# fperezgamonal/flownet2-tf

Measured on AMD Instinct MI355X. Metric: forward pairs/sec at 512x384 (FlowNet2), higher is better.
Workload: dtype f16x2 (split fp16 hi+lo operands, 3 fp16 MFMAs per product, fp32 accumulate); 1 GPU; FlowNet2 forward, batch=4 synthetic 512x384 pairs per GPU, seeded synthetic weights; pairs_per_gpu=4, parallelism=dp1 (no collective)

## Files before the change

flownet2-tf_amd/csrc/conv2.hip:

```cpp
#include "conv_common.h"

#include <type_traits>
#include <algorithm>
#include <utility>

#ifndef FN2_X2_ORDER
#define FN2_X2_ORDER 0
#endif
#ifndef FN2_CONV_ABLATE
#define FN2_CONV_ABLATE 0
#endif
#ifndef FN2_SETPRIO
#define FN2_SETPRIO 1
#endif

namespace fn2 {

typedef __attribute__((address_space(3))) void* lptr_t;

constexpr unsigned kOobOffset = 0x80000000u;

typedef int v4i_t __attribute__((ext_vector_type(4)));
typedef unsigned u32x4_t __attribute__((ext_vector_type(4)));

// ... 476 lines not shown
    issue_stage(lds0);
    asm volatile("s_waitcnt vmcnt(0)" ::: "memory");
    __syncthreads();
    const int nst2 = ((kt1 - (kt0 - grp) + KG - 1) / KG + 1) & ~1;
    for (int s = 0; s < nst2; s += 2) {
      issue_stage(lds1);
      compute(lds0);
      asm volatile("s_waitcnt vmcnt(0)" ::: "memory");
      __syncthreads();
      if (s + 2 < nst2) issue_stage(lds0);
      compute(lds1);
      asm volatile("s_waitcnt vmcnt(0)" ::: "memory");
      __syncthreads();
    }
  } else if constexpr (kDeep) {
    constexpr int ND = NWI + NPI, D = STAGES - 1;
    static_assert(ND * (D - 1) <= 63, "vmcnt field");
    auto slot_ptr = [&](int sl) { return lds0_all + sl * (ROWS * 8); };
#pragma unroll
    for (int d = 0; d < D; ++d) issue_stage(slot_ptr(d));
    const int nst = kt1 - kt0;
    int rd = 0, wr = D;
    for (int s = 0; s < nst; ++s) {
      asm volatile("s_waitcnt vmcnt(%0)\n\ts_barrier" :: "n"(ND * (D - 1)) : "memory");
      issue_stage(slot_ptr(wr));
      compute(slot_ptr(rd));
      rd = rd + 1 == STAGES ? 0 : rd + 1;
      wr = wr + 1 == STAGES ? 0 : wr + 1;
    }
    asm volatile("s_waitcnt vmcnt(0)" ::: "memory");
  } else {
    constexpr int ND = NWI + NPI;
    static_assert(ND == 5 || ND == 6 || ND == 8, "vmcnt literal below");
    auto ring_sync = [] {
      if constexpr (ND == 5) asm volatile("s_waitcnt vmcnt(5)\n\ts_barrier" ::: "memory");
      else if constexpr (ND == 6) asm volatile("s_waitcnt vmcnt(6)\n\ts_barrier" ::: "memory");
      else asm volatile("s_waitcnt vmcnt(8)\n\ts_barrier" ::: "memory");
    };
    issue_stage(lds0);
    issue_stage(lds1);
    const int nst3 = (kt1 - kt0 + 2) / 3 * 3;
    for (int s = 0; s < nst3; s += 3) {
      ring_sync(); issue_stage(lds2); compute(lds0);
      ring_sync(); issue_stage(lds0); compute(lds1);
      ring_sync(); issue_stage(lds1); compute(lds2);
    }
    asm volatile("s_waitcnt vmcnt(0)" ::: "memory");
  }

  if constexpr (KG > 1) {
    constexpr int NA4 = TCN * TPN * 4;
    static_assert((KG - 1) * 4 * NA4 * 64 <= KG * ROWS * 8, "reduction scratch must fit the stage buffers");
    float4* red = reinterpret_cast<float4*>(lds0_all);
    auto acc4 = [&](int idx) -> float4 {
      if constexpr (M16) {
        const f32x4 v = acc16[idx / (TPN * 2)][idx % (TPN * 2)];
        return make_float4(v[0], v[1], v[2], v[3]);
      } else {
        const int t = idx >> 2, q = idx & 3;
        return make_float4(acc[t / TPN][t % TPN][4 * q], acc[t / TPN][t % TPN][4 * q + 1], acc[t / TPN][t % TPN][4 * q + 2],
                           acc[t / TPN][t % TPN][4 * q + 3]);
      }
    };
    if (grp > 0) {
#pragma unroll
      for (int idx = 0; idx < NA4; ++idx) red[(((grp - 1) * 4 + wave) * NA4 + idx) * 64 + lane] = acc4(idx);
    }
    __syncthreads();
    if (grp > 0) return;
#pragma unroll
    for (int g = 0; g < KG - 1; ++g)
#pragma unroll
      for (int idx = 0; idx < NA4; ++idx) {
        const float4 v = red[((g * 4 + wave) * NA4 + idx) * 64 + lane];
        if constexpr (M16) {
          f32x4& d = acc16[idx / (TPN * 2)][idx % (TPN * 2)];
          d[0] += v.x; d[1] += v.y; d[2] += v.z; d[3] += v.w;
        } else {
          const int t = idx >> 2, q = idx & 3;
          acc[t / TPN][t % TPN][4 * q] += v.x; acc[t / TPN][t % TPN][4 * q + 1] += v.y;
          acc[t / TPN][t % TPN][4 * q + 2] += v.z; acc[t / TPN][t % TPN][4 * q + 3] += v.w;
        }
      }
  }

  if constexpr (HEAD5) {
    if (p.dbg & 2) return;
    constexpr int TS = 52;
    static_assert(256 * TS * 4 <= 2 * ROWS * 128, "T fits the stage buffers");
#pragma unroll
    for (int tc = 0; tc < TCN; ++tc)
#pragma unroll
      for (int tp = 0; tp < TPN; ++tp) {
        const int pos = wp * TPN * 32 + tp * 32 + fr;
        const int cb = tc * 32 + fh * 16;
#pragma unroll
        for (int q = 0; q < 4; ++q)
          if (cb + 4 * q < TS)
            *reinterpret_cast<float4*>(h5_t(lds0_all, lds1_all, ROWS * 128, pos * TS + cb + 4 * q)) =
                make_float4(acc[tc][tp][4 * q] * p.out_scale, acc[tc][tp][4 * q + 1] * p.out_scale,
                            acc[tc][tp][4 * q + 2] * p.out_scale, acc[tc][tp][4 * q + 3] * p.out_scale);
      }
    __syncthreads();
    if (p.dbg & 8) return;
    const int tx = bx % p.h5_tx, tyn = bx / p.h5_tx;
    const int n = tyn / p.h5_ty, ty = tyn - n * p.h5_ty;
    float* pf = reinterpret_cast<float*>(p.out);
    if (tid < 224) {
      const int o = tid & 1, px = tid >> 1;
      const int py = px / 28, pxx = px - py * 28;
      const int oy = ty * 4 + py, ox = tx * 28 + pxx;
      if (oy < p.OH && ox < p.OW && !(p.h5_ring && (oy == 0 || oy == p.OH - 1 || ox == 0 || ox == p.OW - 1))) {
        float a = p.bias ? p.bias[o] : 0.f;
#pragma unroll
        for (int uy = 0; uy < 5; ++uy)
#pragma unroll
          for (int ux = 0; ux < 5; ++ux)
            a += *h5_t(lds0_all, lds1_all, ROWS * 128, ((py + uy) * 32 + pxx + ux) * TS + (uy * 5 + ux) * 2 + o);
        pf[(((size_t)n * p.OH + oy) * p.OW + ox) * 2 + o] = a;
      }
    }
    return;
  }
  if (FN2_CONV_ABLATE && (p.dbg & 262144)) return;
  if constexpr (M16) {
    OutT* out16 = reinterpret_cast<OutT*>(p.out);
    const int r16 = lane & 15, g16 = lane >> 4;
    float* slab = p.splitk > 1 ? p.ws + (size_t)split * p.N * p.out_H * p.out_W * p.ws_cs : nullptr;
#pragma unroll
    for (int b = 0; b < TPN * 2; ++b) {
      const int m = m0 + wp * TPN * 32 + b * 16 + r16;
      if (m >= p.M) continue;
      const int n = m / (p.OH * p.OW);
      const int rem = m - n * (p.OH * p.OW);
      const int oy = rem / p.OW, ox = rem - oy * p.OW;
      const size_t opix = ((size_t)n * p.out_H + (oy * osc + oy_off)) * p.out_W + (ox * osc + ox_off);
      OutT* po = out16 + opix * p.out_cs + p.out_c0;
#pragma unroll
      for (int a = 0; a < TCN * 2; ++a) {
        const int co = c0 + wc * TCN * 32 + (a >> 1) * 32 + 16 * (g16 & 1) + 8 * (a & 1) + 4 * (g16 >> 1);
        if (slab != nullptr) {
          if (co < p.ws_cs)
            *reinterpret_cast<float4*>(slab + opix * p.ws_cs + co) =
                make_float4(acc16[a][b][0], acc16[a][b][1], acc16[a][b][2], acc16[a][b][3]);
          continue;
        }
        float v[4];
#pragma unroll
        for (int j = 0; j < 4; ++j) {
          float x = acc16[a][b][j] * p.out_scale + ((p.bias != nullptr && co + j < p.Cout) ? p.bias[co + j] : 0.f);
          if constexpr (sizeof(OutT) == 4) {
            if (p.accum && co + j < p.Cout) x += load_elem<OutT>(po + co + j);
            if (co + j < p.Cout) x = act_grad<OutT>(p, out16, po + co + j, co + j, x);
          }
          if (p.act == FN2_ACT_LEAKY) x = leaky(x);
          v[j] = x;
        }
        if (p.vec_ok && co + 3 < p.Cout) store_vec<OutT, 4>(po + co, v);
        else
#pragma unroll
          for (int j = 0; j < 4; ++j)
            if (co + j < p.Cout) store_elem<OutT>(po + co + j, v[j]);
      }
    }
    return;
  }

  OutT* out = reinterpret_cast<OutT*>(p.out);
  constexpr int WCOLS = TCN * 32, RS = WCOLS + 4, WROWS = 32 * TPN;
  constexpr int WTW = WROWS * RS + WROWS;
  constexpr bool kLdsT = (KG > 1 ? 4 : 2) * WTW * 4 <= KG * ROWS * 128;
  if constexpr (FEED && !kLdsT) { if (feeder) return; }
  float* const tl = reinterpret_cast<float*>(KG > 1 ? ep1 : (wave < 2 ? lds0_all : ep1)) + (KG > 1 ? wave : (wave & 1)) * WTW;
  constexpr int CPR = WCOLS / 4, RPI = 64 / CPR;
  static_assert(!SLAB || WREG, "SLAB is a specialisation of the WREG instantiations");
  if ((SLAB || !WREG) && p.splitk > 1) {
    float* slab = p.ws + (size_t)split * p.N * p.out_H * p.out_W * p.ws_cs;
    if constexpr (kLdsT) {
      if constexpr (STAGES >= 3) __syncthreads();
      if constexpr (FEED) { if (feeder) return; }
      int* rowoff = reinterpret_cast<int*>(tl + WROWS * RS);
#pragma unroll
      for (int tp = 0; tp < TPN; ++tp) {
        const int m = m0 + wp * TPN * 32 + tp * 32 + fr;
        const int mm = m < p.M ? m : 0;
        const int n = mm / (p.OH * p.OW);
        const int rem = mm - n * (p.OH * p.OW);
        const int oy = rem / p.OW, ox = rem - oy * p.OW;
        if (fh == 0) rowoff[tp * 32 + fr] = m < p.M ? (int)((((size_t)n * p.out_H + (oy * osc + oy_off)) * p.out_W + (ox * osc + ox_off)) * p.ws_cs) : -1;
#pragma unroll
        for (int tc = 0; tc < TCN; ++tc)
#pragma unroll
          for (int q = 0; q < 4; ++q)
            *reinterpret_cast<float4*>(tl + (tp * 32 + fr) * RS + tc * 32 + fh * 16 + q * 4) =
                make_float4(acc[tc][tp][4 * q], acc[tc][tp][4 * q + 1], acc[tc][tp][4 * q + 2], acc[tc][tp][4 * q + 3]);
      }
      const int rr = lane / CPR, ch = lane - rr * CPR;
      const int co = c0 + wc * WCOLS + ch * 4;
#pragma unroll
      for (int i = 0; i < WROWS / RPI; ++i) {
        const int row = i * RPI + rr;
        const float4 v = *reinterpret_cast<const float4*>(tl + row * RS + ch * 4);
        const int off = rowoff[row];
        if (off >= 0 && co < p.ws_cs) *reinterpret_cast<float4*>(slab + (size_t)off + co) = v;
      }
      return;
    }
#pragma unroll
    for (int tp = 0; tp < TPN; ++tp) {
      const int m = m0 + wp * TPN * 32 + tp * 32 + fr;
      if (m >= p.M) continue;
      const int n = m / (p.OH * p.OW);
      const int rem = m - n * (p.OH * p.OW);
      const int oy = rem / p.OW, ox = rem - oy * p.OW;
      float* po = slab + (((size_t)n * p.out_H + (oy * osc + oy_off)) * p.out_W + (ox * osc + ox_off)) * p.ws_cs;
#pragma unroll
      for (int tc = 0; tc < TCN; ++tc)
#pragma unroll
        for (int q = 0; q < 4; ++q) {
          const int co = c0 + wc * TCN * 32 + tc * 32 + fh * 16 + q * 4;
          if (co < p.ws_cs)
            *reinterpret_cast<float4*>(po + co) = make_float4(acc[tc][tp][4 * q], acc[tc][tp][4 * q + 1],
                                                              acc[tc][tp][4 * q + 2], acc[tc][tp][4 * q + 3]);
        }
    }
    return;
  }
  if constexpr (SLAB) return;
  const bool vec16 = (p.out_cs % 8 == 0) && (p.out_c0 % 8 == 0);
  const bool wide = kLdsT && sizeof(OutT) == 4 && vec16 && c0 + wc * WCOLS + WCOLS <= p.Cout && !(p.dbg & 4194304);
  int* const rowoff = reinterpret_cast<int*>(tl + WROWS * RS);
  if constexpr (STAGES >= 3 && kLdsT) __syncthreads();
  if constexpr (FEED) { if (feeder) return; }
#pragma unroll
  for (int tc = 0; tc < TCN; ++tc) {
    const int cout_base = c0 + wc * TCN * 32 + tc * 32 + fh * 16;
    float bias[16];
#pragma unroll
    for (int q = 0; q < 16; ++q) bias[q] = (p.bias != nullptr && cout_base + q < p.Cout) ? p.bias[cout_base + q] : 0.f;
#pragma unroll
    for (int tp = 0; tp < TPN; ++tp) {
      const int m = m0 + wp * TPN * 32 + tp * 32 + fr;
      if (wide && tc == 0 && fh == 0) rowoff[tp * 32 + fr] = m < p.M ? 0 : -1;
      if (m >= p.M) continue;
      const int n = m / (p.OH * p.OW);
      const int rem = m - n * (p.OH * p.OW);
      const int oy = rem / p.OW, ox = rem - oy * p.OW;
      const size_t opix = (((size_t)n * p.out_H + (oy * osc + oy_off)) * p.out_W + (ox * osc + ox_off));
      OutT* po = out + opix * p.out_cs + p.out_c0 + cout_base;
      float v[16];
#pragma unroll
      for (int q = 0; q < 16; ++q) v[q] = acc[tc][tp][q] * p.out_scale + bias[q];
      accum_act_grad16<OutT>(p, out, po, cout_base, vec16 && cout_base + 15 < p.Cout, v);
      if (p.act == FN2_ACT_LEAKY) {
#pragma unroll
        for (int q = 0; q < 16; ++q) v[q] = leaky(v[q]);
      }
      if (wide) {
        if (tc == 0 && fh == 0) rowoff[tp * 32 + fr] = (int)opix;
        store16<OutT>(reinterpret_cast<OutT*>(tl + (tp * 32 + fr) * RS + tc * 32 + fh * 16), v);
      } else if (vec16 && cout_base + 15 < p.Cout) {
        store16<OutT>(po, v);
      } else {
#pragma unroll
        for (int q = 0; q < 16; ++q)
          if (cout_base + q < p.Cout) store_elem<OutT>(po + q, v[q]);
      }
    }
  }
  if (wide) {
    const int rr = lane / CPR, ch = lane - rr * CPR;
    OutT* ob = out + p.out_c0 + c0 + wc * WCOLS + ch * 4;
#pragma unroll
    for (int i = 0; i < WROWS / RPI; ++i) {
      const int row = i * RPI + rr;
      const uint4 v = *reinterpret_cast<const uint4*>(tl + row * RS + ch * 4);
      const int opix = rowoff[row];
      if (opix >= 0) *reinterpret_cast<uint4*>(ob + (size_t)opix * p.out_cs) = v;
    }
  }
#endif
}

template <typename OutT, int WC, int WP, int TCN, int TPN, int KW>
__global__ void __launch_bounds__(256) conv_halo_kernel(const ConvArgs p) {
#if defined(__HIP_DEVICE_COMPILE__)
  using T = x2_t;
  constexpr int ESZ = 4;
  constexpr int BC = WC * TCN * 32, BP = WP * TPN * 32;
  static_assert(WC * WP == 4, "4 waves per block");
  constexpr int NWI = BC / 32;
  constexpr int BROWS = BP + 8;
  constexpr int NBP = BROWS / 8;
  constexpr int NBW = (NBP + 3) / 4;
  __shared__ uint4 ldsA[2][BC * 8];
  __shared__ uint4 ldsB[2][BROWS * 8];

  const int tid = threadIdx.x, lane = tid & 63;
  const int wave = __builtin_amdgcn_readfirstlane(tid >> 6);
  const int wc = wave / WP, wp = wave % WP;

  int pad_y = p.pad, pad_x = p.pad, oy_off = 0, ox_off = 0, osc = 1;
  const T* wgt = reinterpret_cast<const T*>(p.wgt);
  const int phase = blockIdx.z;
  const unsigned wrow_bytes = (unsigned)p.ksteps * 128u;
  if (p.merged) {
    pad_y = phase ? p.ph_pad1 : p.ph_pad0; pad_x = 1; oy_off = phase; ox_off = 0; osc = 2;
    wgt += (size_t)phase * p.cout_pad * (wrow_bytes / ESZ);
  } else if (p.deconv) {
    const int a = phase >> 1, b = phase & 1;
    pad_y = a ? p.ph_pad1 : p.ph_pad0; pad_x = b ? p.ph_pad1 : p.ph_pad0; oy_off = a; ox_off = b; osc = 2;
    wgt += (size_t)phase * p.cout_pad * (wrow_bytes / ESZ);
  }
  int bx = blockIdx.x, by = blockIdx.y;
  {
    const int NT = gridDim.x * gridDim.y, L = blockIdx.x + gridDim.x * blockIdx.y;
    const int xcd = L & 7, chunk = NT >> 3, rem = NT & 7;
    const int Lp = xcd * chunk + min(xcd, rem) + (L >> 3);
    bx = Lp / (int)gridDim.y;
    by = Lp - bx * (int)gridDim.y;
  }
  const int m0 = bx * BP, c0 = by * BC;
  const int tn = m0 / (p.OH * p.OW);
  const int trem = m0 - tn * (p.OH * p.OW);
  const int toy = trem / p.OW, tox = trem - toy * p.OW;
  const int iy_base = toy - pad_y, ix_base = tox - pad_x;

  const v4i_t rsrc_w = make_rsrc(wgt, (int)(p.cout_pad * wrow_bytes));
  const v4i_t rsrc_x = make_rsrc(p.in, p.in_bytes);
  const int lrow = lane >> 3, lphys = lane & 7;
  unsigned woff[NWI];
#pragma unroll
  for (int j = 0; j < NWI; ++j) {
    const int row = wave * (BC / 4) + j * 8 + lrow;
    woff[j] = (unsigned)(c0 + row) * wrow_bytes + (unsigned)((lphys ^ ((row >> 1) & 7)) * 16);
  }
  int boff[NBW];
  bool bok[NBW];
#pragma unroll
  for (int j = 0; j < NBW; ++j) {
    const int q = wave + 4 * j;
    const int e = q * 8 + lrow;
    const int ix = ix_base + e;
    bok[j] = q < NBP && e < BP + KW - 1 && ix >= 0 && ix < p.W;
    boff[j] = (((tn * p.H + iy_base) * p.W + ix) * p.in_cs + p.in_c0) * ESZ + (lphys ^ ((e >> 1) & 7)) * 16;
  }
  const int spt = p.cin_chunks >> 3;
  const int nsup = spt * p.KH;
  auto issue_B = [&](int sup, uint4* lds) {
    const int sc = sup / p.KH, ky = sup - sc * p.KH;
    const bool yok = (unsigned)(iy_base + ky) < (unsigned)p.H;
    const int toff = (ky * p.W * p.in_cs) * ESZ + sc * 128;
#pragma unroll
    for (int j = 0; j < NBW; ++j) {
      const int q = wave + 4 * j;
      if (q < NBP) dma16(rsrc_x, &lds[q * 64], (bok[j] && yok) ? (unsigned)(boff[j] + toff) : kOobOffset, 0);
    }
  };
  auto issue_A = [&](int sup, int kx, uint4* lds) {
    const int sc = sup / p.KH, ky = sup - sc * p.KH;
    const int soff = ((ky * KW + kx) * spt + sc) * 128;
#pragma unroll
    for (int j = 0; j < NWI; ++j) dma16(rsrc_w, &lds[(wave * (BC / 4) + j * 8) * 8], woff[j], soff);
  };

  const int fr = lane & 31, fh = lane >> 5, fsw = (fr >> 1) & 7;
  f32x16 acc[TCN][TPN];
#pragma unroll
  for (int tc = 0; tc < TCN; ++tc)
#pragma unroll
    for (int tp = 0; tp < TPN; ++tp)
#pragma unroll
      for (int q = 0; q < 16; ++q) acc[tc][tp][q] = 0.f;

  auto compute = [&](const uint4* la, const uint4* lb, int kx) {
#if FN2_SETPRIO
    __builtin_amdgcn_s_setprio(1);
#endif
    const uint4* A = &la[(wc * TCN * 32 + fr) * 8];
#pragma unroll
    for (int q = 0; q < 2; ++q) {
      const int chh = (4 * q + 2 * fh) ^ fsw, chl = (4 * q + 2 * fh + 1) ^ fsw;
      uint4 ah[TCN], al[TCN], bh[TPN], bl[TPN];
#pragma unroll
      for (int t = 0; t < TCN; ++t) { ah[t] = A[t * 32 * 8 + chh]; al[t] = A[t * 32 * 8 + chl]; }
#pragma unroll
      for (int t = 0; t < TPN; ++t) {
        const int rb = wp * TPN * 32 + t * 32 + fr + kx, sw = (rb >> 1) & 7;
        bh[t] = lb[rb * 8 + ((4 * q + 2 * fh) ^ sw)];
        bl[t] = lb[rb * 8 + ((4 * q + 2 * fh + 1) ^ sw)];
      }
#pragma unroll
      for (int tc = 0; tc < TCN; ++tc)
#pragma unroll
        for (int tp = 0; tp < TPN; ++tp) {
          acc[tc][tp] = mfma_32x32x16<f16_t>(al[tc], bh[tp], acc[tc][tp]);
          acc[tc][tp] = mfma_32x32x16<f16_t>(ah[tc], bl[tp], acc[tc][tp]);
          acc[tc][tp] = mfma_32x32x16<f16_t>(ah[tc], bh[tp], acc[tc][tp]);
        }
    }
#if FN2_SETPRIO
    __builtin_amdgcn_s_setprio(0);
#endif
  };

  issue_B(0, ldsB[0]);
  issue_A(0, 0, ldsA[0]);
  asm volatile("s_waitcnt vmcnt(0)" ::: "memory");
  __syncthreads();
  int abuf = 0;
  for (int sup = 0; sup < nsup; ++sup) {
#pragma unroll
    for (int kx = 0; kx < KW; ++kx) {
      if (kx + 1 < KW) issue_A(sup, kx + 1, ldsA[abuf ^ 1]);
      else if (sup + 1 < nsup) issue_A(sup + 1, 0, ldsA[abuf ^ 1]);
      if (kx == 0 && sup + 1 < nsup) issue_B(sup + 1, ldsB[(sup + 1) & 1]);
      compute(ldsA[abuf], ldsB[sup & 1], kx);
      asm volatile("s_waitcnt vmcnt(0)" ::: "memory");
      __syncthreads();
      abuf ^= 1;
    }
  }

  OutT* out = reinterpret_cast<OutT*>(p.out);
  const bool vec16 = (p.out_cs % 8 == 0) && (p.out_c0 % 8 == 0);
  constexpr int ERS = 36;
  static_assert(sizeof(ldsA) >= 4 * 32 * ERS * 4 || sizeof(ldsB) >= 4 * 32 * ERS * 4, "epilogue tiles fit a stage array");
  float* const etl = reinterpret_cast<float*>(sizeof(ldsA) >= 4 * 32 * ERS * 4 ? &ldsA[0][0] : &ldsB[0][0]) + wave * (32 * ERS);
#pragma unroll
  for (int tc = 0; tc < TCN; ++tc) {
    int cout_base = c0 + wc * TCN * 32 + tc * 32 + fh * 16;
    int bsel = 0;
    if (p.merged) { bsel = cout_base / p.Cout; cout_base -= bsel * p.Cout; if (bsel > 1) continue; }
    float bias[16];
#pragma unroll
    for (int q = 0; q < 16; ++q) bias[q] = (p.bias != nullptr && cout_base + q < p.Cout) ? p.bias[cout_base + q] : 0.f;
#pragma unroll
    for (int tp = 0; tp < TPN; ++tp) {
      const int ox = tox + wp * TPN * 32 + tp * 32 + fr;
      OutT* po = out + (((size_t)tn * p.out_H + (toy * osc + oy_off)) * p.out_W + (ox * osc + ox_off + bsel)) * p.out_cs +
                 p.out_c0 + cout_base;
      float v[16];
#pragma unroll
      for (int q = 0; q < 16; ++q) v[q] = acc[tc][tp][q] * p.out_scale + bias[q];
      accum_act_grad16<OutT>(p, out, po, cout_base, vec16 && cout_base + 15 < p.Cout, v);
      if (p.act == FN2_ACT_LEAKY) {
#pragma unroll
        for (int q = 0; q < 16; ++q) v[q] = leaky(v[q]);
      }
      if (sizeof(OutT) == 4 && vec16 && !p.merged && c0 + wc * TCN * 32 + tc * 32 + 32 <= p.Cout && !(p.dbg & 4194304)) {
        store16<OutT>(reinterpret_cast<OutT*>(etl + fr * ERS + fh * 16), v);
        const int rr = lane >> 3, ch = lane & 7;
        const int ox0 = tox + wp * TPN * 32 + tp * 32;
        OutT* ob = out + (((size_t)tn * p.out_H + (toy * osc + oy_off)) * p.out_W + (ox0 * osc + ox_off)) * p.out_cs +
                   p.out_c0 + c0 + wc * TCN * 32 + tc * 32 + ch * 4;
#pragma unroll
        for (int i = 0; i < 4; ++i) {
          const int row = i * 8 + rr;
          *reinterpret_cast<uint4*>(ob + (size_t)row * osc * p.out_cs) = *reinterpret_cast<const uint4*>(etl + row * ERS + ch * 4);
        }
      } else if (vec16 && cout_base + 15 < p.Cout) {
        store16<OutT>(po, v);
      } else {
#pragma unroll
        for (int q = 0; q < 16; ++q)
          if (cout_base + q < p.Cout) store_elem<OutT>(po + q, v[q]);
      }
      if (p.merged && p.up_src != nullptr && cout_base == 0 && ox < p.OW) {
        const int uy = toy * osc + oy_off, ux = ox * osc + ox_off + bsel;
        const int H2 = p.out_H >> 1, W2 = p.out_W >> 1;
        const int a = uy & 1, b = ux & 1, y = uy >> 1, x = ux >> 1;
        float r0 = p.up_bias ? p.up_bias[0] : 0.f, r1 = p.up_bias ? p.up_bias[1] : 0.f;
#pragma unroll
        for (int ty = 0; ty < 2; ++ty) {
          const int iy = y - 1 + a + ty, ky = 3 - a - 2 * ty;
          if (iy < 0 || iy >= H2) continue;
#pragma unroll
          for (int tx = 0; tx < 2; ++tx) {
            const int ix = x - 1 + b + tx, kx = 3 - b - 2 * tx;
            if (ix < 0 || ix >= W2) continue;
            const float2 sv = *reinterpret_cast<const float2*>(p.up_src + (((long)tn * H2 + iy) * W2 + ix) * 2);
            const float* ww = p.up_w + (ky * 4 + kx) * 4;
            r0 += sv.x * ww[0] + sv.y * ww[1];
            r1 += sv.x * ww[2] + sv.y * ww[3];
          }
        }
        OutT* pu = out + (((size_t)tn * p.out_H + uy) * p.out_W + ux) * p.out_cs + p.up_c0;
        store_elem<OutT>(pu, r0);
        store_elem<OutT>(pu + 1, r1);
      }
    }
  }
#endif
}

template <typename OutT, int NST>
__global__ void __launch_bounds__(256) conv_stem_kernel(const ConvArgs p, const int ntiles) {
#if defined(__HIP_DEVICE_COMPILE__)
  using T = x2_t;
  constexpr int ESZ = 4;
  constexpr int BC = 64, BP = 128, TCN = 2;
  __shared__ uint4 ldsA[NST][BC * 8];
  __shared__ uint4 ldsB[2][NST][BP * 8];
  const int tid = threadIdx.x, lane = tid & 63;
  const int wave = __builtin_amdgcn_readfirstlane(tid >> 6);
  const unsigned wrow_bytes = (unsigned)p.ksteps * 128u;
  const v4i_t rsrc_w = make_rsrc(p.wgt, (int)(p.cout_pad * wrow_bytes));
  const v4i_t rsrc_x = make_rsrc(p.in, p.in_bytes);
  const int lrow = lane >> 3, lphys = lane & 7;
  const int spt = p.cin_chunks >> 3;
#pragma unroll
  for (int st = 0; st < NST; ++st) {
    const int sc = st / p.KH, ky = st - sc * p.KH;
#pragma unroll
    for (int j = 0; j < 2; ++j) {
      const int row = wave * 16 + j * 8 + lrow;
      const unsigned woff = (unsigned)row * wrow_bytes + (unsigned)((lphys ^ ((row >> 1) & 7)) * 16);
      dma16(rsrc_w, &ldsA[st][(wave * 16 + j * 8) * 8], woff, (ky * spt + sc) * 128);
    }
  }
  auto issue_B = [&](int tile, int buf) {
#pragma unroll
    for (int j = 0; j < 4; ++j) {
      const int row = wave * 32 + j * 8 + lrow;
      const int m = tile * BP + row;
      const bool v = m < p.M && tile < ntiles;
      const int mm = v ? m : 0;
      const int n = mm / (p.OH * p.OW);
      const int rem = mm - n * (p.OH * p.OW);
      const int oy = rem / p.OW, ox = rem - oy * p.OW;
      const int roff = (((n * p.H + oy * p.stride) * p.W + ox * p.stride) * p.in_cs + p.in_c0) * ESZ +
                       (lphys ^ ((row >> 1) & 7)) * 16;
#pragma unroll
      for (int st = 0; st < NST; ++st) {
        const int sc = st / p.KH, ky = st - sc * p.KH;
        const int toff = (ky * p.W * p.in_cs) * ESZ + sc * 128;
        dma16(rsrc_x, &ldsB[buf][st][(wave * 32 + j * 8) * 8], v ? (unsigned)(roff + toff) : kOobOffset, 0);
      }
    }
  };
  const int fr = lane & 31, fh = lane >> 5, fsw = (fr >> 1) & 7;
  OutT* out = reinterpret_cast<OutT*>(p.out);
  const bool vec16 = (p.out_cs % 8 == 0) && (p.out_c0 % 8 == 0);
  float bias[TCN][16];
#pragma unroll
  for (int tc = 0; tc < TCN; ++tc)
#pragma unroll
    for (int q = 0; q < 16; ++q) {
      const int co = tc * 32 + fh * 16 + q;
      bias[tc][q] = (p.bias != nullptr && co < p.Cout) ? p.bias[co] : 0.f;
    }

  int tile = blockIdx.x, cur = 0;
  issue_B(tile, 0);
  asm volatile("s_waitcnt vmcnt(0)" ::: "memory");
  __syncthreads();
  for (; tile < ntiles; tile += gridDim.x, cur ^= 1) {
    issue_B(tile + gridDim.x, cur ^ 1);
    f32x16 acc[TCN];
#pragma unroll
    for (int tc = 0; tc < TCN; ++tc)
#pragma unroll
      for (int q = 0; q < 16; ++q) acc[tc][q] = 0.f;
#if FN2_SETPRIO
    __builtin_amdgcn_s_setprio(1);
#endif
#pragma unroll
    for (int st = 0; st < NST; ++st) {
      const uint4* A = &ldsA[st][fr * 8];
      const uint4* B = &ldsB[cur][st][(wave * 32 + fr) * 8];
#pragma unroll
      for (int q = 0; q < 2; ++q) {
        const int chh = (4 * q + 2 * fh) ^ fsw, chl = (4 * q + 2 * fh + 1) ^ fsw;
        const uint4 bh = B[chh], bl = B[chl];
#pragma unroll
        for (int tc = 0; tc < TCN; ++tc) {
          const uint4 ah = A[tc * 32 * 8 + chh], al = A[tc * 32 * 8 + chl];
          acc[tc] = mfma_32x32x16<f16_t>(al, bh, acc[tc]);
          acc[tc] = mfma_32x32x16<f16_t>(ah, bl, acc[tc]);
          acc[tc] = mfma_32x32x16<f16_t>(ah, bh, acc[tc]);
        }
      }
    }
#if FN2_SETPRIO
    __builtin_amdgcn_s_setprio(0);
#endif
    const int m = tile * BP + wave * 32 + fr;
    if (m < p.M) {
      const int n = m / (p.OH * p.OW);
      const int rem = m - n * (p.OH * p.OW);
      const int oy = rem / p.OW, ox = rem - oy * p.OW;
#pragma unroll
      for (int tc = 0; tc < TCN; ++tc) {
        const int cout_base = tc * 32 + fh * 16;
        OutT* po = out + (((size_t)n * p.out_H + oy) * p.out_W + ox) * p.out_cs + p.out_c0 + cout_base;
        float v[16];
#pragma unroll
        for (int q = 0; q < 16; ++q) {
          float x = acc[tc][q] * p.out_scale + bias[tc][q];
          if (p.act == FN2_ACT_LEAKY) x = leaky(x);
          v[q] = x;
        }
        if (vec16 && cout_base + 15 < p.Cout) {
          store16<OutT>(po, v);
        } else {
#pragma unroll
          for (int q = 0; q < 16; ++q)
            if (cout_base + q < p.Cout) store_elem<OutT>(po + q, v[q]);
        }
      }
    }
    asm volatile("s_waitcnt vmcnt(0)" ::: "memory");
    __syncthreads();
  }
#endif
}

template <int CPR>
__global__ void __launch_bounds__(512) head5_strip_kernel(const ConvArgs p) {
#if defined(__HIP_DEVICE_COMPILE__)
  constexpr int RD = 4, CL = 3, NL = CPR * CL;
  constexpr int TS = 68;
  __shared__ uint4 ldsW[NL][64 * 8];
  __shared__ uint4 ldsX[RD][CL][64 * 8];
  __shared__ float T[50 * TS];
  __shared__ float accr[5 * 64 * 2];
  const int tid = threadIdx.x, lane = tid & 63;
  const int wave = __builtin_amdgcn_readfirstlane(tid >> 6);
  const bool feeder = wave >= 4;
  const int w4 = wave & 3;
  const int wc = w4 >> 1, wp = w4 & 1;
  const int H = p.OH, W = p.OW;
  const int nstrip = p.h5_tx, nseg = p.h5_ty, R = p.h5_rows;
  const int b = blockIdx.x;
  const int sx = b % nstrip, sg = (b / nstrip) % nseg, n = b / (nstrip * nseg);
  const int x0 = sx * 60 - 2;
  const int y0 = sg * R, y1 = min(H, y0 + R);
  const int r0 = max(0, y0 - 2), r1 = min(H - 1, y1 + 1);
  const int nch = (r1 - r0 + 1) * CPR;
  const float bias_o[2] = {p.bias ? p.bias[0] : 0.f, p.bias ? p.bias[1] : 0.f};
  const unsigned wrow_bytes = (unsigned)p.ksteps * 128u;
  const v4i_t rsrc_w = make_rsrc(p.wgt, (int)(p.cout_pad * wrow_bytes));
  const v4i_t rsrc_x = make_rsrc(p.in, p.in_bytes);
  const int lrow = lane >> 3, lphys = lane & 7;
  for (int i = tid; i < 5 * 64 * 2; i += 512) accr[i] = 0.f;
  auto issue = [&](int c, int slot) {
    const int rr = c / CPR, kc = c - rr * CPR;
    const int r = r0 + rr;
#pragma unroll
    for (int j = 0; j < 2; ++j) {
      const int px = w4 * 16 + j * 8 + lrow;
      const int x = x0 + px;
      const bool ok = c < nch && x >= 0 && x < W;
      const unsigned off = ok ? (unsigned)((((n * H + r) * W + x) * p.in_cs + p.in_c0) * 4 + (lphys ^ ((px >> 1) & 7)) * 16 +
                                           kc * (CL * 128))
                              : kOobOffset;
#pragma unroll
      for (int ln = 0; ln < CL; ++ln)
        dma16(rsrc_x, &ldsX[slot][ln][(w4 * 16 + j * 8) * 8], ok ? off + ln * 128 : kOobOffset, 0);
    }
  };
  if (feeder) {
#pragma unroll
    for (int ln = 0; ln < NL; ++ln)
#pragma unroll
      for (int j = 0; j < 2; ++j) {
        const int row = w4 * 16 + j * 8 + lrow;
        const unsigned woff = (unsigned)row * wrow_bytes + (unsigned)((lphys ^ ((row >> 1) & 7)) * 16);
        dma16(rsrc_w, &ldsW[ln][(w4 * 16 + j * 8) * 8], woff, ln * 128);
      }
#pragma unroll
    for (int c = 0; c < RD - 1; ++c) issue(c, c);
  }
  const int fr = lane & 31, fh = lane >> 5, fsw = (fr >> 1) & 7;
  float* pf = reinterpret_cast<float*>(p.out);
  f32x16 acc;
  int slot = 0;
  for (int c = 0; c < nch; ++c) {
    const int rr = c / CPR, kc = c - rr * CPR;
    const int r = r0 + rr;
    if (feeder) {
      if constexpr (RD == 5) asm volatile("s_waitcnt vmcnt(18)" ::: "memory");
      else asm volatile("s_waitcnt vmcnt(12)" ::: "memory");
    }
    asm volatile("s_waitcnt lgkmcnt(0)" ::: "memory");
    __builtin_amdgcn_s_barrier();
    const bool last = kc == CPR - 1;
    if (feeder) {
      issue(c + RD - 1, slot == 0 ? RD - 1 : slot - 1);
    } else {
      if (kc == 0) {
#pragma unroll
        for (int q = 0; q < 16; ++q) acc[q] = 0.f;
      }
      if (!(p.dbg & 64))
#pragma unroll
      for (int ln = 0; ln < CL; ++ln) {
        const uint4* A = &ldsW[kc * CL + ln][(wc * 32 + fr) * 8];
        const uint4* B = &ldsX[slot][ln][(wp * 32 + fr) * 8];
#pragma unroll
        for (int q = 0; q < 2; ++q) {
          const int chh = (4 * q + 2 * fh) ^ fsw, chl = (4 * q + 2 * fh + 1) ^ fsw;
          const uint4 bh = B[chh], bl = B[chl];
          const uint4 ah = A[chh], al = A[chl];
          acc = mfma_32x32x16<f16_t>(al, bh, acc);
          acc = mfma_32x32x16<f16_t>(ah, bl, acc);
          acc = mfma_32x32x16<f16_t>(ah, bh, acc);
        }
      }
      if (last) {
        const int cb = wc * 32 + fh * 16;
#pragma unroll
        for (int q = 0; q < 16; ++q)
          if (cb + q < 50) T[(cb + q) * TS + wp * 32 + fr] = acc[q] * p.out_scale;
      }
    }
    asm volatile("s_waitcnt lgkmcnt(0)" ::: "memory");
    __builtin_amdgcn_s_barrier();
    slot = slot == RD - 1 ? 0 : slot + 1;
    if (last && !(p.dbg & 32)) {
      const int x = lane;
      const int xc = min(max(x, 2), 61);
      float tv[2][5], av[2];
      int ai[2];
      bool ok[2], fin[2];
#pragma unroll
      for (int k = 0; k < 2; ++k) {
        const int it = min(wave + 8 * k, 9);
        const int ky = it >> 1, o = it & 1;
        const int y = r + 2 - ky;
        ok[k] = wave + 8 * k < 10 && y >= y0 && y < y1 && x >= 2 && x < 62;
        fin[k] = ky == 4 || r == H - 1;
        const int ys = ((y % 5) + 5) % 5;
        ai[k] = (ys * 64 + xc) * 2 + o;
        const float* t = &T[(ky * 10 + o) * TS + xc - 2];
#pragma unroll
        for (int kx = 0; kx < 5; ++kx) tv[k][kx] = t[2 * kx * TS + kx];
        av[k] = accr[ai[k]];
      }
#pragma unroll
      for (int k = 0; k < 2; ++k) {
        const int it = min(wave + 8 * k, 9);
        const int ky = it >> 1, o = it & 1;
        const int y = r + 2 - ky;
        float sum = tv[k][0];
        sum += tv[k][1];
        sum += tv[k][2];
        sum += tv[k][3];
        sum += tv[k][4];
        const float v = av[k] + sum;
        if (ok[k]) {
          accr[ai[k]] = fin[k] ? 0.f : v;
          const int ox = x0 + x;
          if (fin[k] && ox < W && !(p.h5_ring && (y == 0 || y == H - 1 || ox == 0 || ox == W - 1)))
            pf[(((size_t)n * H + y) * W + ox) * 2 + o] = v + bias_o[o];
        }
      }
    }
  }
  asm volatile("s_waitcnt vmcnt(0)" ::: "memory");
  if (p.h5_wc != nullptr && !(p.dbg & 16)) {
    const long total = (long)p.N * (2 * W + 2 * (H - 2));
    const long per = (total + gridDim.x - 1) / gridDim.x;
    const long m1 = min(total, (long)(b + 1) * per);
    for (long m = (long)b * per + wave; m < m1; m += 8) h5_ring_pixel(p, m);
  }
#endif
}


template <typename OutT, int SPP>
__global__ void __launch_bounds__(256) conv_rowrun_kernel(const ConvArgs p, const int npieces) {
#if defined(__HIP_DEVICE_COMPILE__)
  using T = x2_t;
  constexpr int BC = 64, BP = 128, TCN = 2;
  constexpr int MAXP = SPP == 4 ? 17 : 9;
  __shared__ uint4 ldsA[2][BC * 8];
  __shared__ uint4 ldsB[2][MAXP * 64];
  const int tid = threadIdx.x, lane = tid & 63;
  const int wave = __builtin_amdgcn_readfirstlane(tid >> 6);
  const T* wgt = reinterpret_cast<const T*>(p.wgt);
  const unsigned wrow_bytes = (unsigned)p.ksteps * 128u;
  int bx = blockIdx.x, by = blockIdx.y;
  {
    const int NT = gridDim.x * gridDim.y, L = blockIdx.x + gridDim.x * blockIdx.y;
    const int xcd = L & 7, chunk = NT >> 3, rem = NT & 7;
    const int Lp = xcd * chunk + min(xcd, rem) + (L >> 3);
    bx = Lp / (int)gridDim.y;
    by = Lp - bx * (int)gridDim.y;
  }
  const int m0 = bx * BP, c0 = by * BC;
  const int tn = m0 / (p.OH * p.OW);
  const int trem = m0 - tn * (p.OH * p.OW);
  const int toy = trem / p.OW, tox = trem - toy * p.OW;

  const v4i_t rsrc_w = make_rsrc(wgt, (int)(p.cout_pad * wrow_bytes));
  const v4i_t rsrc_x = make_rsrc(p.in, p.in_bytes);
  const int lrow = lane >> 3, lphys = lane & 7;
  unsigned woff[2];
#pragma unroll
  for (int j = 0; j < 2; ++j) {
    const int row = wave * 16 + j * 8 + lrow;
    woff[j] = (unsigned)(c0 + row) * wrow_bytes + (unsigned)((lphys ^ ((row >> 1) & 7)) * 16);
  }
  const int nslots = ((BP - 1) * p.stride + p.KH_KW_hint) * SPP;
  const int seg0 = (((tn * p.H + toy * p.stride) * p.W + tox * p.stride) * p.in_cs + p.in_c0) * 4;
  constexpr int NBW = (MAXP + 3) / 4;
  unsigned boff[NBW];
#pragma unroll
  for (int j = 0; j < NBW; ++j) {
    const int q = wave + 4 * j;
    const int P = q * 64 + lane;
    const int Ls = P ^ ((P >> 4) & 15);
    boff[j] = (q < npieces && Ls < nslots) ? (unsigned)(seg0 + Ls * 16) : kOobOffset;
  }
  const int nl = p.cin_chunks >> 3;
  const int ngroups = (p.KH_KW_hint * p.in_cs + 7) >> 3;
  auto issue_B = [&](int ky, uint4* lds) {
    const int toff = ky * p.W * p.in_cs * 4;
#pragma unroll
    for (int j = 0; j < NBW; ++j) {
      const int q = wave + 4 * j;
      if (q < npieces) dma16(rsrc_x, &lds[q * 64], boff[j] == kOobOffset ? kOobOffset : boff[j] + (unsigned)toff, 0);
    }
  };
  auto issue_A = [&](int ky, int l, uint4* lds) {
    const int soff = (ky * nl + l) * 128;
#pragma unroll
    for (int j = 0; j < 2; ++j) dma16(rsrc_w, &lds[(wave * 16 + j * 8) * 8], woff[j], soff);
  };

  const int fr = lane & 31, fh = lane >> 5, fsw = (fr >> 1) & 7;
  const int pslot = (wave * 32 + fr) * p.stride * SPP;
  f32x16 acc[TCN];
#pragma unroll
  for (int tc = 0; tc < TCN; ++tc)
#pragma unroll
    for (int q = 0; q < 16; ++q) acc[tc][q] = 0.f;

  issue_B(0, ldsB[0]);
  issue_A(0, 0, ldsA[0]);
  asm volatile("s_waitcnt vmcnt(0)" ::: "memory");
  __syncthreads();
  int abuf = 0;
  for (int ky = 0; ky < p.KH; ++ky) {
    const uint4* lb = ldsB[ky & 1];
    for (int l = 0; l < nl; ++l) {
      if (l + 1 < nl) issue_A(ky, l + 1, ldsA[abuf ^ 1]);
      else if (ky + 1 < p.KH) issue_A(ky + 1, 0, ldsA[abuf ^ 1]);
      if (l == 0 && ky + 1 < p.KH) issue_B(ky + 1, ldsB[(ky + 1) & 1]);
#if FN2_SETPRIO
      __builtin_amdgcn_s_setprio(1);
#endif
      const uint4* A = &ldsA[abuf][fr * 8];
#pragma unroll
      for (int q = 0; q < 2; ++q) {
        if (4 * l + 2 * q >= ngroups) continue;
        const int chh = (4 * q + 2 * fh) ^ fsw, chl = (4 * q + 2 * fh + 1) ^ fsw;
        const int g = 4 * l + 2 * q + fh;
        const int sh = pslot + 2 * g, sl = sh + 1;
        const uint4 bh = lb[sh ^ ((sh >> 4) & 15)], bl = lb[sl ^ ((sl >> 4) & 15)];
#pragma unroll
        for (int tc = 0; tc < TCN; ++tc) {
          const uint4 ah = A[tc * 32 * 8 + chh], al = A[tc * 32 * 8 + chl];
          acc[tc] = mfma_32x32x16<f16_t>(al, bh, acc[tc]);
          acc[tc] = mfma_32x32x16<f16_t>(ah, bl, acc[tc]);
          acc[tc] = mfma_32x32x16<f16_t>(ah, bh, acc[tc]);
        }
      }
#if FN2_SETPRIO
      __builtin_amdgcn_s_setprio(0);
#endif
      asm volatile("s_waitcnt vmcnt(0)" ::: "memory");
      __syncthreads();
      abuf ^= 1;
    }
  }

  OutT* out = reinterpret_cast<OutT*>(p.out);
  const bool vec16 = (p.out_cs % 8 == 0) && (p.out_c0 % 8 == 0);
  const int ox = tox + wave * 32 + fr;
  constexpr int ERS = 36;
  float* const tl = reinterpret_cast<float*>(&ldsB[0][0]) + wave * (32 * ERS);
  static_assert(4 * 32 * ERS * 4 <= (int)sizeof(ldsB), "epilogue tiles fit the segment buffers");
#pragma unroll
  for (int tc = 0; tc < TCN; ++tc) {
    const int cout_base = c0 + tc * 32 + fh * 16;
    OutT* po = out + (((size_t)tn * p.out_H + toy) * p.out_W + ox) * p.out_cs + p.out_c0 + cout_base;
    float v[16];
#pragma unroll
    for (int q = 0; q < 16; ++q) {
      float x = acc[tc][q] * p.out_scale + ((p.bias != nullptr && cout_base + q < p.Cout) ? p.bias[cout_base + q] : 0.f);
      if (p.act == FN2_ACT_LEAKY) x = leaky(x);
      v[q] = x;
    }
    if (sizeof(OutT) == 4 && vec16 && c0 + tc * 32 + 32 <= p.Cout && !(p.dbg & 4194304)) {
      store16<OutT>(reinterpret_cast<OutT*>(tl + fr * ERS + fh * 16), v);
      const int rr = lane >> 3, ch = lane & 7;
      OutT* ob = out + (((size_t)tn * p.out_H + toy) * p.out_W + tox + wave * 32) * p.out_cs + p.out_c0 + c0 + tc * 32 + ch * 4;
#pragma unroll
      for (int i = 0; i < 4; ++i) {
        const int row = i * 8 + rr;
        *reinterpret_cast<uint4*>(ob + (size_t)row * p.out_cs) = *reinterpret_cast<const uint4*>(tl + row * ERS + ch * 4);
      }
    } else if (vec16 && cout_base + 15 < p.Cout) {
      store16<OutT>(po, v);
    } else {
#pragma unroll
      for (int q = 0; q < 16; ++q)
        if (cout_base + q < p.Cout) store_elem<OutT>(po + q, v[q]);
    }
  }
#endif
}

template <typename OutT>
static bool launch_rowrun(const ConvArgs& a, int tile, int phases, hipStream_t s) {
  if ((a.dbg & 65536) || tile != 64 || phases != 1 || a.deconv || a.KW != 1 || a.KH_KW_hint < 1 || a.splitk != 1 || a.accum || a.wfrag)
    return false;
  if (a.OW % 128 != 0 || (a.in_cs != 8 && a.in_cs != 16)) return false;
  const int spp = a.in_cs / 4;
  const int nl = a.cin_chunks >> 3;
  const int max_slot = 127 * a.stride * spp + 2 * (4 * nl - 1) + 1;
  const int npieces = max_slot / 64 + 1;
  if (npieces > (spp == 4 ? 17 : 9)) return false;
  dim3 grid(a.M / 128, a.cout_pad / 64, 1), block(256);
  if (conv_name_sink().buf) {
    snprintf(conv_name_sink().buf, conv_name_sink().cap, "conv_rowrun_kernel<%s, %d>", is_x2<OutT>::value ? "fn2::x2_t" : "float", spp);
    return true;
  }
  if (spp == 4) hipLaunchKernelGGL((conv_rowrun_kernel<OutT, 4>), grid, block, 0, s, a, npieces);
  else hipLaunchKernelGGL((conv_rowrun_kernel<OutT, 2>), grid, block, 0, s, a, npieces);
  return true;
}

template <typename OutT>
static bool launch_stem(const ConvArgs& a, int tile, int phases, hipStream_t s) {
  if ((a.dbg & 8192) || tile != 64 || phases != 1 || a.deconv || a.KW != 1 || a.splitk != 1 || a.accum ||
      a.ksteps < 1 || a.ksteps > 4 || a.cout_pad != 64)
    return false;
  const int ntiles = cdiv(a.M, 128);
  if (ntiles < 512) return false;
  const char* e = getenv("FN2_STEM_BLOCKS");
  const int blocks = std::min(ntiles, e ? atoi(e) : 256);
  if (conv_name_sink().buf) {
    snprintf(conv_name_sink().buf, conv_name_sink().cap, "conv_stem_kernel<%s, %d>",
             is_x2<OutT>::value ? "fn2::x2_t" : "float", a.ksteps);
    return true;
  }
  switch (a.ksteps) {
    case 1: hipLaunchKernelGGL((conv_stem_kernel<OutT, 1>), dim3(blocks), dim3(256), 0, s, a, ntiles); break;
    case 2: hipLaunchKernelGGL((conv_stem_kernel<OutT, 2>), dim3(blocks), dim3(256), 0, s, a, ntiles); break;
    case 3: hipLaunchKernelGGL((conv_stem_kernel<OutT, 3>), dim3(blocks), dim3(256), 0, s, a, ntiles); break;
    default: hipLaunchKernelGGL((conv_stem_kernel<OutT, 4>), dim3(blocks), dim3(256), 0, s, a, ntiles); break;
  }
  return true;
}

template <typename OutT>
static bool launch_halo(const ConvArgs& a, int tile, int phases, hipStream_t s) {
  if (((a.dbg & 2048) && !a.merged) || a.stride != 1 || a.splitk != 1 || a.kg != 1 || !a.bp64 || a.wfrag || (a.KW != 2 && a.KW != 3)) return false;
  if (a.deconv && (a.kh_ph[0] != a.KH || a.kh_ph[1] != a.KH || a.kw_ph[0] != a.KW || a.kw_ph[1] != a.KW)) return false;
  if (tile == 128 && a.bp64 == 2 && !(a.dbg & 4096)) return false;
  if (a.bp64 == 3) return false;
  const int bp = tile == 128 ? 64 : 128;
  if (a.OW % bp != 0 || a.M % bp != 0) return false;
  dim3 block(256);
#define FN2_HALO(GY, ...)                                                                         \
  do {                                                                                            \
    dim3 grid(a.M / bp, GY, phases);                                                              \
    if (conv_name_sink().buf)                                                                     \
      snprintf(conv_name_sink().buf, conv_name_sink().cap, "conv_halo_kernel<%s, %s, %d>",       \
               is_x2<OutT>::value ? "fn2::x2_t" : "float", #__VA_ARGS__, a.KW);                    \
    else if (a.KW == 3) hipLaunchKernelGGL((conv_halo_kernel<OutT, __VA_ARGS__, 3>), grid, block, 0, s, a); \
    else hipLaunchKernelGGL((conv_halo_kernel<OutT, __VA_ARGS__, 2>), grid, block, 0, s, a);      \
  } while (0)
  if (tile == 128) FN2_HALO(a.cout_pad / 128, 2, 2, 2, 1);
  else if (tile == 64) FN2_HALO(a.cout_pad / 64, 1, 4, 2, 1);
  else FN2_HALO(a.cout_pad / 32, 1, 4, 1, 1);
#undef FN2_HALO
  return true;
}

template <typename T> static const char* type_name();
template <> const char* type_name<float>() { return "float"; }
template <> const char* type_name<bf16_t>() { return "__bf16"; }
template <> const char* type_name<f16_t>() { return "_Float16"; }
template <> const char* type_name<x2_t>() { return "fn2::x2_t"; }

ConvNameSink& conv_name_sink() {
  static thread_local ConvNameSink sink{nullptr, 0};
  return sink;
}

template <typename T, typename OutT>
static int launch2(const ConvArgs& a, int tile, int phases, hipStream_t s) {
  const int z = phases * a.splitk;
  const long blocks64 = (long)cdiv(a.M, 64) * (a.cout_pad / 128) * z;
  const char* e_m16 = getenv("FN2_M16_MIN");
  const bool m16 = is_x2<T>::value && !(a.dbg & 512) &&
                   ((a.dbg & 1024) || (e_m16 && tile == 128 && a.bp64 == 1 && a.kg == 1 && a.splitk == 1 &&
                                       blocks64 >= atoi(e_m16)));
#define FN2_LAUNCH2(GX, GY, THREADS, ...)                                                              \
  do {                                                                                                 \
    dim3 grid(GX, GY, z);                                                                              \
    if (conv_name_sink().buf)                                                                          \
      snprintf(conv_name_sink().buf, conv_name_sink().cap, "conv_igemm2_kernel<%s, %s, %s, %s>", type_name<T>(), \
               type_name<OutT>(), #__VA_ARGS__, m16 ? "true" : "false");                              \
    else if (m16) hipLaunchKernelGGL((conv_igemm2_kernel<T, OutT, __VA_ARGS__, is_x2<T>::value>), grid, dim3(THREADS), 0, s, a); \
    else hipLaunchKernelGGL((conv_igemm2_kernel<T, OutT, __VA_ARGS__, false>), grid, dim3(THREADS), 0, s, a);            \
  } while (0)
  if (a.wfrag) {
    if constexpr (is_x2<T>::value) {
      if (tile == 64) {
        dim3 grid(cdiv(a.M, 128), a.cout_pad / 64, z);
        if (conv_name_sink().buf)
          snprintf(conv_name_sink().buf, conv_name_sink().cap, "conv_igemm2_kernel<%s, %s, 2, 2, 1, 2, 2, 1, false, true, %s>",
                   type_name<T>(), type_name<OutT>(), a.splitk > 1 ? "true" : "false");
        else if (a.splitk > 1)
          hipLaunchKernelGGL((conv_igemm2_kernel<T, OutT, 2, 2, 1, 2, 2, 1, false, true, true>), grid, dim3(256), 0, s, a);
        else
          hipLaunchKernelGGL((conv_igemm2_kernel<T, OutT, 2, 2, 1, 2, 2, 1, false, true, false>), grid, dim3(256), 0, s, a);
      } else {
        dim3 grid(cdiv(a.M, 64), a.cout_pad / 128, z);
        const bool slab = a.splitk > 1;
        ConvArgs ah = a;
        if (a.fh_M > 0 && slab && !conv_name_sink().buf) {
          const char* e = getenv("FN2_FH_BLOCKS");
          const long per_z = (long)grid.x * grid.y;
          const long want = std::min<long>(a.fh_M, e ? atoi(e) : 1024);
          ah.fh_z0 = z;
          grid.z = z + (unsigned)std::max<long>(1, (want + per_z - 1) / per_z);
        } else {
          ah.fh_M = 0;
        }
        const ConvArgs& a = ah;
        const char* e_feed = getenv("FN2_WREG_FEED");
        const int feed = e_feed ? atoi(e_feed) : 1;
        if (conv_name_sink().buf)
          snprintf(conv_name_sink().buf, conv_name_sink().cap, "conv_igemm2_kernel<%s, %s, 4, 1, 1, 2, %d, 1, false, true, %s%s>",
                   type_name<T>(), type_name<OutT>(), a.wfrag == 2 ? 3 : 2, slab ? "true" : "false",
                   (a.wfrag == 2 && (slab ? feed >= 2 : feed >= 1)) ? ", false, true" : "");
        else if (a.wfrag == 2 && slab && feed >= 2)
          hipLaunchKernelGGL((conv_igemm2_kernel<T, OutT, 4, 1, 1, 2, 3, 1, false, true, true, false, true>), grid, dim3(512), 0, s, a);
        else if (a.wfrag == 2 && slab)
          hipLaunchKernelGGL((conv_igemm2_kernel<T, OutT, 4, 1, 1, 2, 3, 1, false, true, true>), grid, dim3(256), 0, s, a);
        else if (a.wfrag == 2 && feed >= 1)
          hipLaunchKernelGGL((conv_igemm2_kernel<T, OutT, 4, 1, 1, 2, 3, 1, false, true, false, false, true>), grid, dim3(512), 0, s, a);
        else if (a.wfrag == 2)
          hipLaunchKernelGGL((conv_igemm2_kernel<T, OutT, 4, 1, 1, 2, 3, 1, false, true, false>), grid, dim3(256), 0, s, a);
        else if (slab)
          hipLaunchKernelGGL((conv_igemm2_kernel<T, OutT, 4, 1, 1, 2, 2, 1, false, true, true>), grid, dim3(256), 0, s, a);
        else
          hipLaunchKernelGGL((conv_igemm2_kernel<T, OutT, 4, 1, 1, 2, 2, 1, false, true, false>), grid, dim3(256), 0, s, a);
      }
    } else {
      return fail(FN2_ERR_UNSUPPORTED, "conv fast path: fragment-order weights are split fp16 only");
    }
  } else if (tile == 128 && a.bp64 && a.kg == 3) FN2_LAUNCH2(cdiv(a.M, 64), a.cout_pad / 128, 768, 2, 2, 2, 1, 2, 3);
  else if (tile == 128 && a.bp64 && a.kg == 2) FN2_LAUNCH2(cdiv(a.M, 64), a.cout_pad / 128, 512, 2, 2, 2, 1, 2, 2);
  else if (tile == 128 && a.bp64 == 3) FN2_LAUNCH2(cdiv(a.M, 64), a.cout_pad / 128, 256, 2, 2, 2, 1, 6, 1);
  else if (tile == 128 && a.bp64 == 2) FN2_LAUNCH2(cdiv(a.M, 64), a.cout_pad / 128, 256, 2, 2, 2, 1, 3, 1);
  else if (tile == 128 && a.bp64) FN2_LAUNCH2(cdiv(a.M, 64), a.cout_pad / 128, 256, 2, 2, 2, 1, 2, 1);
  else if (tile == 128) FN2_LAUNCH2(cdiv(a.M, 128), a.cout_pad / 128, 256, 2, 2, 2, 2, 2, 1);
  else if (tile == 64 && a.bp64) FN2_LAUNCH2(cdiv(a.M, 128), a.cout_pad / 64, 256, 1, 4, 2, 1, 2, 1);
  else if (tile == 64) FN2_LAUNCH2(cdiv(a.M, 256), a.cout_pad / 64, 256, 1, 4, 2, 2, 2, 1);
  else if (a.bp64) FN2_LAUNCH2(cdiv(a.M, 128), a.cout_pad / 32, 256, 1, 4, 1, 1, 2, 1);
  else FN2_LAUNCH2(cdiv(a.M, 256), a.cout_pad / 32, 256, 1, 4, 1, 2, 2, 1);
#undef FN2_LAUNCH2
  FN2_CHECK_LAUNCH("conv_igemm2");
  return FN2_OK;
}

int launch_head5_strip(const ConvArgs& a, int blocks, hipStream_t s) {
  if (a.ksteps == 3) hipLaunchKernelGGL((head5_strip_kernel<1>), dim3(blocks), dim3(512), 0, s, a);
  else if (a.ksteps == 6) hipLaunchKernelGGL((head5_strip_kernel<2>), dim3(blocks), dim3(512), 0, s, a);
  else return fail(FN2_ERR_UNSUPPORTED, "flow_head5 strip form: %d channel lines (3 or 6)", a.ksteps);
  FN2_CHECK_LAUNCH("flow_head5_strip");
  return FN2_OK;
}

int launch_head5(const ConvArgs& a, int blocks, hipStream_t s) {
  hipLaunchKernelGGL((conv_igemm2_kernel<x2_t, float, 1, 4, 2, 2, 2, 1, false, false, false, true>), dim3(blocks, 1, 1), dim3(256), 0,
                     s, a);
  FN2_CHECK_LAUNCH("flow_head5");
  return FN2_OK;
}

bool conv_fast_ok(int in_dtype, int cin_pad, int cout) {
  const int esz = dtype_size(in_dtype);
  return cout > 2 && (cin_pad * esz) % 128 == 0;
}

int launch_conv_fast(const ConvArgs& a, int in_dtype, int out_dtype, int tile, int phases, hipStream_t s) {
  if (tile != 128 && tile != 64 && tile != 32) return fail(FN2_ERR_UNSUPPORTED, "conv fast path: cout tile %d", tile);
  if (in_dtype == FN2_F32) return launch2<float, float>(a, tile, phases, s);
  if (in_dtype == FN2_BF16) {
    if (out_dtype == FN2_BF16) return launch2<bf16_t, bf16_t>(a, tile, phases, s);
    return launch2<bf16_t, float>(a, tile, phases, s);
  }
  if (in_dtype == FN2_F16) {
    if (out_dtype == FN2_F16) return launch2<f16_t, f16_t>(a, tile, phases, s);
    return launch2<f16_t, float>(a, tile, phases, s);
  }
  if (out_dtype == FN2_F16X2) {
    if (launch_rowrun<x2_t>(a, tile, phases, s)) { FN2_CHECK_LAUNCH("conv_rowrun"); return FN2_OK; }
    if (launch_stem<x2_t>(a, tile, phases, s)) { FN2_CHECK_LAUNCH("conv_stem"); return FN2_OK; }
    if (launch_halo<x2_t>(a, tile, phases, s)) { FN2_CHECK_LAUNCH("conv_halo"); return FN2_OK; }
    if (a.merged) return fail(FN2_ERR_UNSUPPORTED, "conv2d kind 5: needs the halo kernel (input width a multiple of 128, no split-K)");
    return launch2<x2_t, x2_t>(a, tile, phases, s);
  }
  if (launch_halo<float>(a, tile, phases, s)) { FN2_CHECK_LAUNCH("conv_halo"); return FN2_OK; }
  if (a.merged) return fail(FN2_ERR_UNSUPPORTED, "conv2d kind 5: needs the halo kernel (input width a multiple of 128, no split-K)");
  return launch2<x2_t, float>(a, tile, phases, s);
}

}
```

Measured before the change: 1102 pairs/s.

## Let halo conv tiles span multiple output rows and fold deconv phases into grid

The halo convolution kernel can now cover small-width feature maps (OW dividing 128) by packing several output rows into one 128-pixel tile, loading a halo strip per row and remapping fragment and epilogue addresses. Layers that previously fell back to a generic path can use the halo kernel. Deconvolution phases are also folded into the linearized XCD-swizzled block index instead of gridDim.z, so phases of the same tile land near each other. This adds per-lane row bookkeeping and wastes some LDS rows at row boundaries.

```diff
diff --git a/flownet2-tf_amd/csrc/conv2.hip b/flownet2-tf_amd/csrc/conv2.hip
--- a/flownet2-tf_amd/csrc/conv2.hip
+++ b/flownet2-tf_amd/csrc/conv2.hip
@@ -802,7 +802,17 @@
 
   int pad_y = p.pad, pad_x = p.pad, oy_off = 0, ox_off = 0, osc = 1;
   const T* wgt = reinterpret_cast<const T*>(p.wgt);
-  const int phase = blockIdx.z;
+  const int nph = (p.deconv && gridDim.z == 1) ? (p.merged ? 2 : 4) : 1;
+  int bx, by, phase = blockIdx.z;
+  {
+    const int NT = gridDim.x * gridDim.y, L = blockIdx.x + gridDim.x * blockIdx.y;
+    const int xcd = L & 7, chunk = NT >> 3, rem = NT & 7;
+    const int Lp = xcd * chunk + min(xcd, rem) + (L >> 3);
+    int t = Lp;
+    if (nph > 1) { t = Lp / nph; phase = Lp - t * nph; }
+    bx = t / (int)gridDim.y;
+    by = t - bx * (int)gridDim.y;
+  }
   const unsigned wrow_bytes = (unsigned)p.ksteps * 128u;
   if (p.merged) {
     pad_y = phase ? p.ph_pad1 : p.ph_pad0; pad_x = 1; oy_off = phase; ox_off = 0; osc = 2;
@@ -812,19 +822,15 @@
     pad_y = a ? p.ph_pad1 : p.ph_pad0; pad_x = b ? p.ph_pad1 : p.ph_pad0; oy_off = a; ox_off = b; osc = 2;
     wgt += (size_t)phase * p.cout_pad * (wrow_bytes / ESZ);
   }
-  int bx = blockIdx.x, by = blockIdx.y;
-  {
-    const int NT = gridDim.x * gridDim.y, L = blockIdx.x + gridDim.x * blockIdx.y;
-    const int xcd = L & 7, chunk = NT >> 3, rem = NT & 7;
-    const int Lp = xcd * chunk + min(xcd, rem) + (L >> 3);
-    bx = Lp / (int)gridDim.y;
-    by = Lp - bx * (int)gridDim.y;
-  }
   const int m0 = bx * BP, c0 = by * BC;
   const int tn = m0 / (p.OH * p.OW);
   const int trem = m0 - tn * (p.OH * p.OW);
   const int toy = trem / p.OW, tox = trem - toy * p.OW;
   const int iy_base = toy - pad_y, ix_base = tox - pad_x;
+  const int tw = min(p.OW, BP);
+  const int tsh = __builtin_ctz(tw);
+  const int lw = tw + KW - 1;
+  const int lend = (BP >> tsh) * lw;
 
   const v4i_t rsrc_w = make_rsrc(wgt, (int)(p.cout_pad * wrow_bytes));
   const v4i_t rsrc_x = make_rsrc(p.in, p.in_bytes);
@@ -835,25 +841,27 @@
     const int row = wave * (BC / 4) + j * 8 + lrow;
     woff[j] = (unsigned)(c0 + row) * wrow_bytes + (unsigned)((lphys ^ ((row >> 1) & 7)) * 16);
   }
-  int boff[NBW];
+  int boff[NBW], biy[NBW];
   bool bok[NBW];
 #pragma unroll
   for (int j = 0; j < NBW; ++j) {
     const int q = wave + 4 * j;
     const int e = q * 8 + lrow;
-    const int ix = ix_base + e;
-    bok[j] = q < NBP && e < BP + KW - 1 && ix >= 0 && ix < p.W;
-    boff[j] = (((tn * p.H + iy_base) * p.W + ix) * p.in_cs + p.in_c0) * ESZ + (lphys ^ ((e >> 1) & 7)) * 16;
+    const int rr = (e >= lw) + (e >= 2 * lw) + (e >= 3 * lw);
+    const int ix = ix_base + e - rr * lw;
+    bok[j] = q < NBP && e < lend && ix >= 0 && ix < p.W;
+    biy[j] = iy_base + rr;
+    boff[j] = (((tn * p.H + biy[j]) * p.W + ix) * p.in_cs + p.in_c0) * ESZ + (lphys ^ ((e >> 1) & 7)) * 16;
   }
   const int spt = p.cin_chunks >> 3;
   const int nsup = spt * p.KH;
   auto issue_B = [&](int sup, uint4* lds) {
     const int sc = sup / p.KH, ky = sup - sc * p.KH;
-    const bool yok = (unsigned)(iy_base + ky) < (unsigned)p.H;
     const int toff = (ky * p.W * p.in_cs) * ESZ + sc * 128;
 #pragma unroll
     for (int j = 0; j < NBW; ++j) {
       const int q = wave + 4 * j;
+      const bool yok = (unsigned)(biy[j] + ky) < (unsigned)p.H;
       if (q < NBP) dma16(rsrc_x, &lds[q * 64], (bok[j] && yok) ? (unsigned)(boff[j] + toff) : kOobOffset, 0);
     }
   };
@@ -872,6 +880,12 @@
     for (int tp = 0; tp < TPN; ++tp)
 #pragma unroll
       for (int q = 0; q < 16; ++q) acc[tc][tp][q] = 0.f;
+  int srow[TPN], sfrag[TPN];
+#pragma unroll
+  for (int t = 0; t < TPN; ++t) {
+    srow[t] = (wp * TPN * 32 + t * 32) >> tsh;
+    sfrag[t] = wp * TPN * 32 + t * 32 + srow[t] * (KW - 1);
+  }
 
   auto compute = [&](const uint4* la, const uint4* lb, int kx) {
 #if FN2_SETPRIO
@@ -886,7 +900,7 @@
       for (int t = 0; t < TCN; ++t) { ah[t] = A[t * 32 * 8 + chh]; al[t] = A[t * 32 * 8 + chl]; }
 #pragma unroll
       for (int t = 0; t < TPN; ++t) {
-        const int rb = wp * TPN * 32 + t * 32 + fr + kx, sw = (rb >> 1) & 7;
+        const int rb = sfrag[t] + fr + kx, sw = (rb >> 1) & 7;
         bh[t] = lb[rb * 8 + ((4 * q + 2 * fh) ^ sw)];
         bl[t] = lb[rb * 8 + ((4 * q + 2 * fh + 1) ^ sw)];
       }
@@ -937,8 +951,10 @@
     for (int q = 0; q < 16; ++q) bias[q] = (p.bias != nullptr && cout_base + q < p.Cout) ? p.bias[cout_base + q] : 0.f;
 #pragma unroll
     for (int tp = 0; tp < TPN; ++tp) {
-      const int ox = tox + wp * TPN * 32 + tp * 32 + fr;
-      OutT* po = out + (((size_t)tn * p.out_H + (toy * osc + oy_off)) * p.out_W + (ox * osc + ox_off + bsel)) * p.out_cs +
+      const int oy = toy + srow[tp];
+      const int ox0 = tox + wp * TPN * 32 + tp * 32 - (srow[tp] << tsh);
+      const int ox = ox0 + fr;
+      OutT* po = out + (((size_t)tn * p.out_H + (oy * osc + oy_off)) * p.out_W + (ox * osc + ox_off + bsel)) * p.out_cs +
                  p.out_c0 + cout_base;
       float v[16];
 #pragma unroll
@@ -951,8 +967,7 @@
       if (sizeof(OutT) == 4 && vec16 && !p.merged && c0 + wc * TCN * 32 + tc * 32 + 32 <= p.Cout && !(p.dbg & 4194304)) {
         store16<OutT>(reinterpret_cast<OutT*>(etl + fr * ERS + fh * 16), v);
         const int rr = lane >> 3, ch = lane & 7;
-        const int ox0 = tox + wp * TPN * 32 + tp * 32;
-        OutT* ob = out + (((size_t)tn * p.out_H + (toy * osc + oy_off)) * p.out_W + (ox0 * osc + ox_off)) * p.out_cs +
+        OutT* ob = out + (((size_t)tn * p.out_H + (oy * osc + oy_off)) * p.out_W + (ox0 * osc + ox_off)) * p.out_cs +
                    p.out_c0 + c0 + wc * TCN * 32 + tc * 32 + ch * 4;
 #pragma unroll
         for (int i = 0; i < 4; ++i) {
@@ -967,7 +982,7 @@
           if (cout_base + q < p.Cout) store_elem<OutT>(po + q, v[q]);
       }
       if (p.merged && p.up_src != nullptr && cout_base == 0 && ox < p.OW) {
-        const int uy = toy * osc + oy_off, ux = ox * osc + ox_off + bsel;
+        const int uy = oy * osc + oy_off, ux = ox * osc + ox_off + bsel;
         const int H2 = p.out_H >> 1, W2 = p.out_W >> 1;
         const int a = uy & 1, b = ux & 1, y = uy >> 1, x = ux >> 1;
         float r0 = p.up_bias ? p.up_bias[0] : 0.f, r1 = p.up_bias ? p.up_bias[1] : 0.f;
@@ -1464,11 +1479,13 @@
   if (tile == 128 && a.bp64 == 2 && !(a.dbg & 4096)) return false;
   if (a.bp64 == 3) return false;
   const int bp = tile == 128 ? 64 : 128;
-  if (a.OW % bp != 0 || a.M % bp != 0) return false;
+  const bool rows = bp == 128 && !a.merged && !(a.dbg & 8388608) && a.OW >= 32 && bp % a.OW == 0 && (a.OH * a.OW) % bp == 0;
+  if ((a.OW % bp != 0 && !rows) || a.M % bp != 0) return false;
+  const bool fold = a.deconv && !(a.dbg & 16777216);
   dim3 block(256);
 #define FN2_HALO(GY, ...)                                                                         \
   do {                                                                                            \
-    dim3 grid(a.M / bp, GY, phases);                                                              \
+    dim3 grid(a.M / bp * (fold ? phases : 1), GY, fold ? 1 : phases);                             \
     if (conv_name_sink().buf)                                                                     \
       snprintf(conv_name_sink().buf, conv_name_sink().cap, "conv_halo_kernel<%s, %s, %d>",       \
                is_x2<OutT>::value ? "fn2::x2_t" : "float", #__VA_ARGS__, a.KW);                    \
```

Result: no change. 1107 pairs/s, median of 6 (+0.4%).
